# refresh-bio/fqsqueezer

Hardware: AMD Instinct MI355X
Metric: Mbases/s compressed (DNA stream, SE sorted) (higher is better)
Workload: dtype u64; 1 GPU; 1000000x150bp SE, G=7500000 (seed 2+rank), -om s -gs 8 -qm n -im n; workers_T=64, blocks=256, per_gpu=one independent file per GPU

## Files before the change

### fqsqueezer_amd/csrc/fqsx_api.hip

```cpp
#include "fqsx_kernels.h"
#include "fqsx_qual.h"
#include "fqsx_qdec.h"
#include "../../include/fqsx.h"
#include "fqsx_vm.h"
#include "fqsx_rt.h"
#include <sys/resource.h>

#ifndef FQSX_EMU
#include <dlfcn.h>
#include <rccl/rccl.h>
#endif
#include <algorithm>
#include <cstdio>
#include <cstdlib>
#include <cstring>
#include <string>
#include <vector>

extern "C" const char *fqsx_last_error(void) { return g_err.c_str(); }
extern "C" const char *fqsx_version(void) {
#ifdef FQSX_EMU
  return "fqsx 0.1 (host emulation build - tests only)";
#else
  return "fqsx 0.1 (HIP gfx950)";
// ... 30 lines not shown
    for (u64 i = first; i < nb_slots; i += stride) cfg.l_b.slots[i] = 0;
    for (u64 i = first; i < ns_slots; i += stride) cfg.l_s.slots[i] = 0;
    for (u64 i = first; i < 2ull * cfg.T; i += stride) cfg.l_s.filled[i] = 0;
    return;
  }
  insert_phase_body(cfg, &sm, FQ_BLOCK / 3, FQ_BLOCK % 3, win, maxmult, by_source != 0);
  if (cfg.sys_scope) fq_release_system();
}
FQ_KERNEL64 void k_compact_generic(const u8 *out, u64 out_cap, const u64 *lens, u8 *dst) {
  const u32 tid = FQ_BLOCK;
  u64 off = 0;
  for (u32 t = 0; t < tid; ++t) off += lens[t];
  const u64 n = lens[tid] <= out_cap ? lens[tid] : 0;
  const u8 *src = out + (u64)tid * out_cap;
  for (u64 i = FQ_LANE; i < n; i += FQ_WAVE) dst[off + i] = src[i];
}
FQ_KERNEL64 void k_clear_local(DevCfg cfg, u64 nb_slots, u64 ns_slots) {
  if (phase_skip(cfg)) return;
  const u64 stride = (u64)FQ_NBLOCKS * FQ_WAVE, first = (u64)FQ_BLOCK * FQ_WAVE + FQ_LANE;
  for (u64 i = first; i < nb_slots; i += stride) cfg.l_b.slots[i] = 0;
  for (u64 i = first; i < ns_slots; i += stride) cfg.l_s.slots[i] = 0;
  for (u64 i = first; i < 2ull * cfg.T; i += stride) cfg.l_s.filled[i] = 0;
}
FQ_KERNEL64 void k_finish_block(DevCfg cfg, u64 *lens , u64 *end ) {
  if (FQ_LANE == 0) {
    if (FQ_BLOCK == 0) { end[2 * cfg.T] = cfg.err[0]; end[2 * cfg.T + 1] = cfg.err[1]; }
    if (cfg.err[1]) return;
    finish_block_body(cfg, FQ_BLOCK);
    lens[FQ_BLOCK] = cfg.ws[FQ_BLOCK].out_len;
    end[FQ_BLOCK] = cfg.ws[FQ_BLOCK].out_len;
// ... 467 lines not shown
    u8 *va = nullptr;
    u64 va_bytes = 0, chunk_bytes = 0;
    std::vector<fqsx_vm::Handle> h;
    std::vector<u8> mapped;
    u64 own_bytes = 0;
    u32 own_mod = 0;
    bool live = false;
  } vm_s, vm_b, vm_pk, vm_pv, vm_siv;
  u32 *d_plog_n;
  u32 ins_win, ins_maxmult;
  bool part_sender;
  bool defer_coding;
  u64 gq_entries;
  u32 gq_test_cap;
  bool cur_defer;
  u64 vm_own_bytes;
};

namespace {

#define FQSX_PIN_BYTES (64u * 1024u)
int d2h_small_begin(fqsx_dna *c, const void *d, u64 bytes) { return d2h(c, c->h_pin, d, bytes); }
int d2h_small_end(fqsx_dna *c, void *h, u64 bytes) {
  DEVCHK(dev_sync(c));
  memcpy(h, c->h_pin, bytes);
  return FQSX_OK;
}

#define REHASH_GRID FQ_GRID(2048)

// ... 347 lines not shown
  int rc = dev_launch(c, 0, true, [&] {
#ifndef FQSX_EMU
    if (defer) return fqsx_launch_encode_se_defer(c->stream, a);
#endif
    return decode ? fqsx_launch_decode(c->stream, a) : c->paired ? fqsx_launch_encode_pe(c->stream, a) : fqsx_launch_encode_se(c->stream, a);
  });
#ifndef FQSX_EMU
  if (!rc && defer) {
    if (c->profiling) rc = dev_launch(c, 2, true, [&] { return fqsx_launch_code_se(c->stream, a); });
    else if (!(rc = dev_side_launch(c, buf, [&] { return fqsx_launch_code_se(c->side, a); }))) c->k_n[2] += 1;
  }
#endif
  return rc;
}

int block_prepare(fqsx_dna *c, const u8 *d_bases, const u64 *d_off, const u64 *h_off, u32 n_reads, u32 generation,
                  const u8 *const *dec_streams = nullptr, const u64 *dec_lens = nullptr) {
  const bool decode = dec_streams != nullptr;
  const u32 T = c->T;
  DevCfg &cfg = c->cfg;
  u64 S = generation < 100u ? 100u - generation : 0u;
  u64 cap_s = (u64)n_reads / T / 2;
  if (S > cap_s) S = cap_s;
  if (S) --S;
  u64 max_wbases = 0, max_seg_bases = 0, max_seg_reads = 0, max_wreads = 0, max_defer_entries = 0;
  DEVCHK(dev_side_join(c));
  std::vector<u64> wbases(T);
  for (u32 t = 0; t < T; ++t) {
    u64 first, last;
    worker_reads(t, T, n_reads, first, last);
    wbases[t] = h_off[last] - h_off[first];
    max_wbases = std::max(max_wbases, wbases[t]);
// ... 5 lines not shown
        const u64 ns = segment_synchro(seg, S, first, last);
        if (!c->paired) stop = ns + 1;
        else { u64 i = cur; if (i < ns) i += (ns - i + 1) & ~1ull; stop = i + 2; }
      }
      if (stop > last) stop = last;
      if (stop > cur) {
        max_seg_bases = std::max(max_seg_bases, h_off[stop] - h_off[cur]);
        max_seg_reads = std::max(max_seg_reads, stop - cur);
        if (seg < S) max_defer_entries = std::max(max_defer_entries, h_off[stop] - h_off[cur] + (stop - cur) * (FQSX_HD_RAW + 0u));
        cur = stop;
      }
    }
  }
  int rc;
  void *p = nullptr;
  if (c->paired && (n_reads & 1)) { g_err = "paired-end blocks need an even number of reads"; return FQSX_E_ARG; }
  u64 need_out = max_wbases + 16 * max_wreads + 1024;
  if ((rc = dfit(c, cfg.out, cfg.out_cap, need_out, pow2_at_least(need_out), T))) return rc;
  const u64 mail_entries[3] = {2 * max_seg_bases + 2 * max_seg_reads, max_seg_bases, 2 * max_seg_bases};
  for (u32 k = 0; k < 3; ++k) {
    u64 need = mail_entries[k] + 64;
    if (need > c->mail_cap[k] && (rc = mail_alloc(c, k, (u32)(need + need / 4)))) return rc;
  }
  u64 need_lb = pow2_at_least(4 * max_seg_bases + 64), need_ls = pow2_at_least(2 * max_seg_bases + 64);
  if ((rc = ltab_fit(c, cfg.l_b, c->lb_cap, need_lb, cfg.bmer, 6))) return rc;
  if ((rc = ltab_fit(c, cfg.l_s, c->ls_cap, need_ls, cfg.smer, 12))) return rc;
  u64 need_lpe = 0;
  if (c->paired) {
    const u64 seg_pairs = max_seg_reads / 2 + 1;
    const u64 need_list = 14 * seg_pairs + 16;
    const u32 list_cap = (u32)(need_list + need_list / 4);
    if ((rc = dfit(c, cfg.pe_bkt, c->pe_bkt_cap, need_list, list_cap, (u64)T * 3 * sizeof(u64)))) return rc;
    if ((rc = dfit(c, cfg.pe_list, cfg.pe_cap, need_list, list_cap, (u64)T * 3 * sizeof(u64)))) return rc;
// ... 152 lines not shown
int pe_insert_and_clear(fqsx_dna *c) {
  LAUNCH(c, 2, k_pe_insert, c->T, 64, c->cfg);
  return pe_clear_local(c);
}

int block_segment(fqsx_dna *c, u32 seg) {
  const u32 T = c->T, n_reads = c->cur_n_reads;
  const u64 S = c->cur_S, need_lpe = c->cur_need_lpe;
  const bool decode = c->cur_decode;
  DevCfg &cfg = c->cfg;
  int rc;
  {
    const bool defer = c->cur_defer && seg < S;
    if (!defer) DEVCHK(dev_side_join(c));
    if ((rc = launch_segment(c, decode, n_reads, (u32)S, seg, defer))) return rc;
    const u32 part_grid = T * (cfg.mail[0].n_tiles + cfg.mail[1].n_tiles + cfg.mail[2].n_tiles);
    if (!decode && c->part_sender) LAUNCH(c, 2, k_part_sender, 3 * T, FQSX_SND_THREADS, cfg);
    else {
      LAUNCH(c, 2, k_part_count, part_grid, 64, cfg);
      LAUNCH(c, 2, k_part_scan, 3 * T, 64, cfg);
      if (!decode) LAUNCH(c, 2, k_part_scatter, part_grid, 64, cfg, seg + 1, c->d_demand);
    }
    if (!decode) {
      if (c->paired) {
        const u32 bgrid = FQ_GRID((u32)std::min<u64>(1024, ((u64)T * cfg.pe_cap + 255) / 256));
        LAUNCH(c, 2, k_pe_bucket_count, bgrid, 256, cfg);
        LAUNCH(c, 2, k_pe_bucket_offsets, 1, 64, cfg, seg + 1);
        LAUNCH(c, 2, k_pe_bucket_scatter, bgrid, 256, cfg);
        LAUNCH(c, 2, k_pe_insert_buckets, T, 64, cfg);
        if ((rc = pe_clear_local(c))) return rc;
// ... 8 lines not shown
      g_err = "device error " + std::to_string(c->h_demand[2 * T]) + " in decode kernel (block " + std::to_string(c->cur_gen) + ")";
      return FQSX_E_DEVICE;
    }
    if ((rc = grow_for_demand(c))) return rc;
    if (c->paired) {
      LAUNCH(c, 2, k_pe_demand, T, 64, cfg, c->d_demand, 0u);
      if ((rc = d2h_sync(c, c->h_demand.data(), c->d_demand, T * sizeof(u32)))) return rc;
      if ((rc = d2h_sync(c, c->h_filled.data(), cfg.g_pe.filled, T * sizeof(u32)))) return rc;
      u64 need = 0;
      for (u32 o = 0; o < T; ++o) need = std::max<u64>(need, (u64)c->h_filled[o] + c->h_demand[o]);
      if (need * 2 > c->gpe_cap && (rc = grow_gpe(c, pow2_at_least(need * 2 + 2)))) return rc;
      if ((rc = pe_insert_and_clear(c))) return rc;
    }
    LAUNCH(c, 1, k_insert_phase, 3 * T, FQSX_INS_THREADS, cfg, (u64)0, (u64)0, c->ins_win, c->ins_maxmult, 0u, 0u);
    if ((rc = clear_local_tables(c))) return rc;
  }
  return FQSX_OK;
}

int block_finish(fqsx_dna *c, const u64 *h_off, const u8 **streams, u64 *lens, u8 *bases_out, u32 *posted = nullptr) {
  if (posted) *posted = 0;
  const u32 T = c->T, n_reads = c->cur_n_reads, generation = c->cur_gen;
  const bool decode = c->cur_decode;
  DevCfg &cfg = c->cfg;
  int rc;
  if (decode) {
    u32 derr = 0;
    if ((rc = d2h_sync(c, &derr, cfg.err, sizeof(u32)))) return rc;
    if (derr) {
      g_err = "device error " + std::to_string(derr) + " while decoding block " + std::to_string(generation);
      return FQSX_E_DEVICE;
    }
    return bases_out ? d2h_sync(c, bases_out, cfg.dout, h_off[n_reads]) : FQSX_OK;
  }
  DEVCHK(dev_side_join(c));
  LAUNCH(c, 2, k_finish_block, T, 64, cfg, c->d_lens, c->d_end);
  {
    std::vector<u64> e(2 * T + 2);
    if ((rc = d2h_small_begin(c, c->d_end, e.size() * sizeof(u64)))) return rc;
    if ((rc = d2h_small_end(c, e.data(), e.size() * sizeof(u64)))) return rc;
    if (e[2 * T]) {
      g_err = "device error " + std::to_string(e[2 * T]) + " while encoding block " + std::to_string(generation);
      return FQSX_E_DEVICE;
    }
    if (e[2 * T + 1]) {
      if (posted) { *posted = (u32)e[2 * T + 1]; return FQSX_OK; }
      g_err = "growth posted by the device outside the deferred path";
      return FQSX_E_DEVICE;
    }
    for (u32 t = 0; t < T; ++t) { c->h_lens[t] = e[t]; c->h_filled[t] = (u32)e[T + t]; }
    c->filled_valid = true;
  }
  u64 total = 0;
  for (u32 t = 0; t < T; ++t) {
    if (c->h_lens[t] > cfg.out_cap) { g_err = "stream overflow"; return FQSX_E_DEVICE; }
    total += c->h_lens[t];
  }
  if ((rc = dfit(c, c->d_compact, c->compact_cap, total, total + total / 2 + 4096, 1))) return rc;
  return collect_streams(c, c->d_compact, T, cfg.out, cfg.out_cap, c->d_lens, c->h_lens, c->h_out, streams, lens);
}

int encode_block_impl(fqsx_dna *c, const u8 *d_bases, const u64 *d_off, const u64 *h_off, u32 n_reads, u32 generation,
                      const u8 **streams, u64 *lens, const u8 *const *dec_streams = nullptr, const u64 *dec_lens = nullptr,
                      u8 *bases_out = nullptr) {
  if (c->shard_world > 1) { g_err = "a sharded codec is driven through fqsx_shard_* (fqsqueezer_amd/sharded.py)"; return FQSX_E_ARG; }
  int rc = block_prepare(c, d_bases, d_off, h_off, n_reads, generation, dec_streams, dec_lens);
  for (u32 seg = 0; !rc;) {
    for (; !rc && seg <= c->cur_S; ++seg) rc = block_segment(c, seg);
    u32 posted = 0;
    if (!rc) rc = block_finish(c, h_off, streams, lens, bases_out, &posted);
    if (rc || !posted) break;
    rc = block_recover(c, posted - 1);
    seg = posted;
  }
  return rc;
}

bool defer_possible(fqsx_dna *c, u32 n_parts) {
#ifdef FQSX_EMU
  (void)c; (void)n_parts;
  return false;
// ... 134 lines not shown
  }
  cfg.shard_rank = 0; cfg.shard_world = 1; cfg.shard_cnt = nullptr;
  if ((rc = dalloc(c, &p, sizeof(u32) * 4, true))) return rc;
  cfg.err = (u32 *)p;
#ifdef FQSX_TIMING
  if ((rc = dalloc(c, &p, (u64)FQSX_TRACE_LAUNCHES * T * FQSX_TRACE_W * sizeof(u64), true))) return rc;
  cfg.trace = (u64 *)p;
#endif
  if ((rc = dalloc(c, &p, (5 * (u64)T + 2) * sizeof(u32), true))) return rc;
  c->d_demand = cfg.demand = (u32 *)p;
  if ((rc = dalloc(c, &p, ((u64)T + 64) * sizeof(u64), true))) return rc;
  c->d_lens = (u64 *)p;
  if ((rc = dalloc(c, &p, (2 * (u64)T + 2) * sizeof(u64), true))) return rc;
  c->d_end = (u64 *)p;
  if ((rc = pinned_alloc((void **)&c->h_pin, FQSX_PIN_BYTES))) return rc;
  c->h_demand.assign(4 * T + 1, 0);
  c->h_filled.assign(T, 0);
  c->h_lens.assign(T + 64, 0);
  DEVCHK(dev_sync(c));
  return FQSX_OK;
}

}

extern "C" {

int fqsx_dna_create(const uint8_t *h, int device, fqsx_dna **out) { return fqsx_dna_create_on_partition(h, device, 0, 1, out); }

int fqsx_dna_create_on_partition(const uint8_t *h, int device, uint32_t part, uint32_t n_parts, fqsx_dna **out) {
  if (n_parts == 0 || part >= n_parts) { g_err = "bad compute-unit partition"; return FQSX_E_ARG; }
// ... 16 lines not shown
  }
  rc = create_impl(c, h);
  if (!rc) c->defer_coding = defer_possible(c, n_parts);
  if (!rc && getenv("FQSX_CHUNKED_TABLES") && atoi(getenv("FQSX_CHUNKED_TABLES"))) rc = fqsx_dna_use_chunked_tables(c);
  if (rc) {
    fqsx_dna_destroy(c);
    return rc;
  }
  *out = c;
  return FQSX_OK;
}

void fqsx_dna_destroy(fqsx_dna *c) {
  if (!c) return;
  dev_close(c);
  vtab_free(c, c->vm_s);
  vtab_free(c, c->vm_b);
  vtab_free(c, c->vm_pk);
  vtab_free(c, c->vm_pv);
  vtab_free(c, c->vm_siv);
  fqsx_vm::mesh_close(c->mesh);
  pinned_free(c->h_pin);
  delete c;
}

int fqsx_dna_encode_block_dev(fqsx_dna *c, const uint8_t *d_bases, const uint64_t *d_off, const uint64_t *h_off,
                              uint32_t n_reads, uint32_t generation, const uint8_t **streams, uint64_t *lens) {
  if (!c || !d_bases || !d_off || !h_off || !streams || !lens) { g_err = "null argument"; return FQSX_E_ARG; }
  DEVCHK(dev_enter(c));
  return encode_block_impl(c, d_bases, d_off, h_off, n_reads, generation, streams, lens);
}

int fqsx_dna_encode_block(fqsx_dna *c, const uint8_t *bases, const uint64_t *off, uint32_t n_reads, uint32_t generation,
                          const uint8_t **streams, uint64_t *lens) {
  if (!c || !bases || !off || !streams || !lens) { g_err = "null argument"; return FQSX_E_ARG; }
  DEVCHK(dev_enter(c));
  int rc;
  u64 nb = off[n_reads] + 64, no = ((u64)n_reads + 1) * sizeof(u64);
  if ((rc = dfit(c, c->d_bases, c->dev_bases_cap, nb, nb + nb / 4, 1))) return rc;
  if ((rc = dfit(c, c->d_off, c->dev_off_cap, no, no + no / 4, 1))) return rc;
  if ((rc = h2d(c, c->d_bases, bases, off[n_reads]))) return rc;
  if ((rc = h2d(c, c->d_off, off, no))) return rc;
  return encode_block_impl(c, c->d_bases, c->d_off, off, n_reads, generation, streams, lens);
}

static int decode_args_ok(const fqsx_dna *c, const uint8_t *const *streams, const uint64_t *lens, const uint64_t *off, uint32_t n_reads) {
  if (c->paired && (n_reads & 1)) { g_err = "paired-end blocks need an even number of reads"; return FQSX_E_ARG; }
  if (off[0] != 0) { g_err = "read offsets do not start at 0"; return FQSX_E_ARG; }
  for (uint32_t i = 0; i < n_reads; ++i) {
    if (off[i + 1] < off[i]) { g_err = "read offsets do not ascend"; return FQSX_E_ARG; }
    if (off[i + 1] - off[i] >= (1ull << 24)) { g_err = "a read of 2^24 bases or more"; return FQSX_E_ARG; }
  }
  for (uint32_t t = 0; t < c->T; ++t)
    if (lens[t] && !streams[t]) { g_err = "null stream"; return FQSX_E_ARG; }
  return FQSX_OK;
}

int fqsx_dna_decode_block(fqsx_dna *c, const uint8_t *const *streams, const uint64_t *lens, const uint64_t *off, uint32_t n_reads,
                          uint32_t generation, uint8_t *bases_out) {
  if (!c || !streams || !lens || !off || !bases_out) { g_err = "null argument"; return FQSX_E_ARG; }
  if (int bad = decode_args_ok(c, streams, lens, off, n_reads)) return bad;
  DEVCHK(dev_enter(c));
  int rc;
  u64 no = ((u64)n_reads + 1) * sizeof(u64);
  if ((rc = dfit(c, c->d_off, c->dev_off_cap, no, no + no / 4, 1))) return rc;
  if ((rc = h2d(c, c->d_off, off, no))) return rc;
  return encode_block_impl(c, nullptr, c->d_off, off, n_reads, generation, nullptr, nullptr, streams, lens, bases_out);
}

int fqsx_dna_decode_block_dev(fqsx_dna *c, const uint8_t *const *streams, const uint64_t *lens, const uint64_t *off, uint32_t n_reads,
                              uint32_t generation, const uint8_t **d_bases_out) {
  if (d_bases_out) *d_bases_out = nullptr;
  if (!c || !streams || !lens || !off || !d_bases_out) { g_err = "null argument"; return FQSX_E_ARG; }
  if (int bad = decode_args_ok(c, streams, lens, off, n_reads)) return bad;
  DEVCHK(dev_enter(c));
  int rc;
  u64 no = ((u64)n_reads + 1) * sizeof(u64);
  if ((rc = dfit(c, c->d_off, c->dev_off_cap, no, no + no / 4, 1))) return rc;
  if ((rc = h2d(c, c->d_off, off, no))) return rc;
  if ((rc = encode_block_impl(c, nullptr, c->d_off, off, n_reads, generation, nullptr, nullptr, streams, lens, nullptr))) return rc;
  *d_bases_out = c->cfg.dout;
  return FQSX_OK;
}

int fqsx_shard_config(fqsx_dna *c, uint32_t rank, uint32_t world) {
  if (!c || world == 0 || rank >= world || world > c->T) { g_err = "bad rank / world size"; return FQSX_E_ARG; }
  if (c->part && world > 1) { g_err = "a codec with chunked tables cannot be sharded afterwards (fqsx_shard_partition_tables after the attach)"; return FQSX_E_ARG; }
  DEVCHK(dev_enter(c));
  const u32 T = c->T;
  c->shard_rank = rank; c->shard_world = world;
  c->cfg.shard_rank = rank; c->cfg.shard_world = world;
  u8 vm[256];
  for (u32 i = 0; i < 256; ++i) vm[i] = (u8)i;
  u32 v = 0;
  for (u32 q = 0; q < world; ++q)
    for (u32 o = q; o < T; o += world) vm[o] = (u8)v++;
  int rc;
  void *p = nullptr;
  if ((rc = h2d(c, c->d_vmap, vm, 256))) return rc;
  if (!c->cfg.shard_cnt) {
    if ((rc = dalloc(c, &p, (3ull * T * T + T + 1) * sizeof(u32), true))) return rc;
    c->cfg.shard_cnt = (u32 *)p;
    if ((rc = dalloc(c, &p, (3ull * T * T + T + 1) * sizeof(u32), true))) return rc;
// ... 1 lines not shown
    if ((rc = dalloc(c, &p, 3ull * (T + 1) * T * sizeof(u32), true))) return rc;
    c->d_colsum = (u32 *)p;
    if ((rc = dalloc(c, &p, 8 * sizeof(u64), true))) return rc;
    c->d_small = (u64 *)p;
    c->h_cglob.assign(3ull * T * T + T + 1, 0);
  }
  DEVCHK(dev_sync(c));
  return FQSX_OK;
}

int fqsx_shard_begin_block(fqsx_dna *c, const uint8_t *bases , const uint64_t *off , const uint64_t *h_off,
                           uint32_t n_reads, uint32_t generation, uint32_t *n_segments) {
  if (!c || !bases || !off || !h_off || !n_segments) { g_err = "null argument"; return FQSX_E_ARG; }
  if (c->part) { g_err = "partitioned tables are driven through fqsx_shard_encode_block"; return FQSX_E_ARG; }
  if (c->paired && c->shard_world > 1) { g_err = "paired-end files are sharded through fqsx_shard_attach + fqsx_shard_encode_block (the step-wise fqsx_shard_* driver does not exchange the pair-table triples)"; return FQSX_E_ARG; }
  DEVCHK(dev_enter(c));
  int rc = block_prepare(c, bases, off, h_off, n_reads, generation);
  *n_segments = c->cur_S + 1;
  return rc;
}

int fqsx_shard_encode(fqsx_dna *c, uint32_t seg, uint32_t *counts ) {
  if (!c || !counts) { g_err = "null argument"; return FQSX_E_ARG; }
  DEVCHK(dev_enter(c));
  const u32 T = c->T;
  DevCfg &cfg = c->cfg;
  int rc;
  if ((rc = launch_segment(c, false, c->cur_n_reads, c->cur_S, seg))) return rc;
  const u32 part_grid = T * (cfg.mail[0].n_tiles + cfg.mail[1].n_tiles + cfg.mail[2].n_tiles);
  LAUNCH(c, 2, k_part_count, part_grid, 64, cfg);
  LAUNCH(c, 2, k_shard_counts, 3 * T + 1, 64, cfg, cfg.shard_cnt, 0u);
  if ((rc = d2d(c, counts, cfg.shard_cnt, 3ull * T * T * sizeof(u32)))) return rc;
  u32 err = 0;
  if ((rc = d2h_sync(c, &err, cfg.err, sizeof(u32)))) return rc;
  if (err) { g_err = "device error " + std::to_string(err) + " in encode kernel"; return FQSX_E_DEVICE; }
  return FQSX_OK;
}

int fqsx_shard_pack(fqsx_dna *c, const uint32_t *counts_sum , uint64_t *const send[3] ) {
  if (!c || !counts_sum || !send) { g_err = "null argument"; return FQSX_E_ARG; }
  DEVCHK(dev_enter(c));
  const u32 T = c->T;
  DevCfg &cfg = c->cfg;
  int rc;
  if ((rc = d2d(c, c->d_cglob, counts_sum, 3ull * T * T * sizeof(u32)))) return rc;
  const u32 part_grid = T * (cfg.mail[0].n_tiles + cfg.mail[1].n_tiles + cfg.mail[2].n_tiles);
  LAUNCH(c, 2, k_part_scan, 3 * T, 64, cfg);
  LAUNCH(c, 2, k_part_dstoff, 3, 64, cfg, c->d_demand, 0u);
  LAUNCH(c, 2, k_part_scatter, part_grid, 64, cfg, 0u, (u32 *)nullptr);
  std::vector<u32> tot(3 * (T + 1));
  for (u32 k = 0; k < 3; ++k)
    if ((rc = d2h_sync(c, tot.data() + k * (T + 1), cfg.mail[k].dst_off, (T + 1) * sizeof(u32)))) return rc;
  for (u32 k = 0; k < 3; ++k) {
    const u64 n = tot[k * (T + 1) + T];
    if (n && (rc = d2d(c, send[k], cfg.mail[k].sorted, n * sizeof(u64)))) return rc;
  }
  DEVCHK(dev_sync(c));
  return FQSX_OK;
}

int fqsx_shard_merge(fqsx_dna *c, const uint64_t *const recv[3] , uint64_t need[2]) {
  if (!c || !recv || !need) { g_err = "null argument"; return FQSX_E_ARG; }
  DEVCHK(dev_enter(c));
  const u32 T = c->T;
  DevCfg &cfg = c->cfg;
  int rc;
  for (u32 k = 0; k < 3; ++k) LAUNCH(c, 2, k_shard_merge, T, 64, cfg, k, recv[k], (const u32 *)c->d_cglob);
  need[0] = need[1] = 0;
  std::vector<u32> tot(T), fil(T);
  for (int which = 0; which < 2; ++which) {
    const KTab &t = which ? cfg.g_b : cfg.g_s;
    if ((rc = d2h_sync(c, tot.data(), cfg.mail[which ? MAIL_B : MAIL_S].dst_tot, T * sizeof(u32)))) return rc;
    if ((rc = d2h_sync(c, fil.data(), t.filled, T * sizeof(u32)))) return rc;
    for (u32 o = 0; o < T; ++o) need[which] = std::max<u64>(need[which], (u64)tot[o] + fil[o]);
  }
  return FQSX_OK;
}

int fqsx_shard_insert(fqsx_dna *c, uint64_t need_s, uint64_t need_b, uint64_t *const items[3] , uint64_t siv_delta[2]) {
  if (!c || !items || !siv_delta) { g_err = "null argument"; return FQSX_E_ARG; }
  DEVCHK(dev_enter(c));
  const u32 T = c->T;
  DevCfg &cfg = c->cfg;
  int rc;
  if (tab_over(c, need_s, c->gs_cap) && (rc = grow_global(c, cfg.g_s, c->gs_cap, tab_new_cap(c, need_s)))) return rc;
  if (tab_over(c, need_b, c->gb_cap) && (rc = grow_global(c, cfg.g_b, c->gb_cap, tab_new_cap(c, need_b)))) return rc;
  if ((rc = d2h_sync(c, c->siv_before, cfg.siv_stats, 2 * sizeof(u64)))) return rc;
  LAUNCH(c, 1, k_insert_phase, 3 * T, FQSX_INS_THREADS, cfg, (u64)0, (u64)0, c->ins_win, c->ins_maxmult, 0u, 0u);
  u64 after[2];
  if ((rc = d2h_sync(c, after, cfg.siv_stats, 2 * sizeof(u64)))) return rc;
  siv_delta[0] = after[0] - c->siv_before[0];
  siv_delta[1] = after[1] - c->siv_before[1];
  for (u32 k = 0; k < 3; ++k) LAUNCH(c, 2, k_shard_collect, REHASH_GRID, 256, cfg, k, items[k]);
  DEVCHK(dev_sync(c));
  return FQSX_OK;
}

int fqsx_shard_apply(fqsx_dna *c, uint32_t kind, const uint64_t *items , uint64_t n) {
  if (!c || kind > 2 || (!items && n)) { g_err = "bad argument"; return FQSX_E_ARG; }
  DEVCHK(dev_enter(c));
  if (n) LAUNCH(c, 2, k_shard_apply, REHASH_GRID, 256, c->cfg, kind, items, (u32)n);
  return FQSX_OK;
}

int fqsx_shard_end_phase(fqsx_dna *c, const uint64_t siv_delta_sum[2]) {
  if (!c || !siv_delta_sum) { g_err = "null argument"; return FQSX_E_ARG; }
  DEVCHK(dev_enter(c));
  int rc;
  u64 now[2] = {c->siv_before[0] + siv_delta_sum[0], c->siv_before[1] + siv_delta_sum[1]};
  if ((rc = h2d(c, c->cfg.siv_stats, now, 2 * sizeof(u64)))) return rc;
  DEVCHK(dev_sync(c));
  return clear_local_tables(c);
}

int fqsx_shard_finish_block(fqsx_dna *c, const uint64_t *h_off, const uint8_t **streams, uint64_t *lens) {
  if (!c || !h_off || !streams || !lens) { g_err = "null argument"; return FQSX_E_ARG; }
  DEVCHK(dev_enter(c));
  return block_finish(c, h_off, streams, lens, nullptr);
}

namespace {
int xbuf_fit(fqsx_dna *c, u64 *&buf, u64 &cap, u64 words) { return dfit(c, buf, cap, words, words + words / 4 + 1024, sizeof(u64)); }
#define COMMCHK(x, what) do { if ((x) != 0) { if (g_err.empty() || g_err.find(what) == std::string::npos) g_err = std::string(what) + " failed"; if (c->comm.abort) c->comm.abort(c->comm.ctx); return FQSX_E_HIP; } } while (0)

int shard_vote(fqsx_dna *c, int fail, const char *what) {
  const u64 NC = 3ull * c->T * c->T + c->T + 1;
  u32 *word = c->d_cglob + NC - 1;
  u32 v = fail ? 1u : 0u;
  const std::string mine = g_err;
  int rc;
  if ((rc = h2d(c, word, &v, sizeof(v)))) return rc;
  DEVCHK(dev_sync(c));
// ... 181 lines not shown
      c->cfg.siv = (u64 *)c->vm_siv.va;
      c->cfg.siv_part = 1;
      void *p = nullptr;
      if ((rc = dalloc(c, &p, 2 * sizeof(u32), true))) return rc;
      c->d_plog_n = (u32 *)p;
      c->cfg.p_log_n = c->d_plog_n;
    }
  }
  DEVCHK(dev_sync(c));
  return FQSX_OK;
}
}

int fqsx_dna_use_chunked_tables(fqsx_dna *c) {
  if (!c) { g_err = "null argument"; return FQSX_E_ARG; }
  if (c->part) return FQSX_OK;
  if (c->k_n[0] || c->shard_world > 1) { g_err = "chunked tables are chosen before the first block (sharded codecs: fqsx_shard_partition_tables)"; return FQSX_E_ARG; }
  DEVCHK(dev_enter(c));
  return tables_to_chunks(c);
}

int fqsx_shard_partition_tables(fqsx_dna *c) {
  if (!c || !c->comm_set) { g_err = "no transport attached (fqsx_shard_attach)"; return FQSX_E_ARG; }
  if (c->part && (c->shard_world == 1 || !c->mesh.peer.empty())) return FQSX_OK;
  if (c->part || c->k_n[0]) { g_err = "the tables can only be partitioned before the first block"; return FQSX_E_ARG; }
  DEVCHK(dev_enter(c));
  const u32 G = c->shard_world, me = c->shard_rank;
  int rc;
  c->part_fallback = false;
#ifndef FQSX_EMU
  if (G > 1) {
    u64 mine[2] = {0, 0};
    char bus[16] = {0};
    HIPCHK(hipDeviceGetPCIBusId(bus, (int)sizeof(bus), c->device));
    memcpy(mine, bus, sizeof(mine));
    std::vector<u64> all(2ull * G, 0);
    if ((rc = xbuf_fit(c, c->d_items, c->items_cap, 2))) return rc;
    if ((rc = xbuf_fit(c, c->d_gathered, c->gathered_cap, 2ull * G))) return rc;
    if ((rc = h2d(c, c->d_items, mine, sizeof(mine)))) return rc;
    DEVCHK(dev_sync(c));
    COMMCHK(c->comm.allgather_u64(c->comm.ctx, c->d_items, 2, c->d_gathered), "all-gather of the ranks' PCI bus ids");
// ... 27 lines not shown
  if ((rc = xbuf_fit(c, c->d_gathered, c->gathered_cap, G))) return rc;
  if ((rc = h2d(c, c->d_items, &c->mesh.word, sizeof(u64)))) return rc;
  COMMCHK(c->comm.allgather_u64(c->comm.ctx, c->d_items, 1, c->d_gathered), "all-gather of the descriptor-socket names");
  if ((rc = d2h_sync(c, words.data(), c->d_gathered, G * sizeof(u64)))) return rc;
  VMCHK(fqsx_vm::mesh_connect(c->mesh, words.data(), e_));
  if ((rc = tables_to_chunks(c))) return rc;
  COMMCHK(c->comm.allgather_u64(c->comm.ctx, c->d_items, 1, c->d_gathered), "barrier after the table partition");
  DEVCHK(dev_sync(c));
  return FQSX_OK;
}

int fqsx_shard_encode_block(fqsx_dna *c, const uint8_t *bases, const uint64_t *off, const uint64_t *h_off, uint32_t n_reads,
                            uint32_t generation, const uint8_t **streams, uint64_t *lens) {
  if (!c || !bases || !off || !h_off || !streams || !lens) { g_err = "null argument"; return FQSX_E_ARG; }
  if (!c->comm_set) { g_err = "no transport attached (fqsx_shard_attach)"; return FQSX_E_ARG; }
  DEVCHK(dev_enter(c));
  int rc = block_prepare(c, bases, off, h_off, n_reads, generation);
  for (u32 seg = 0; !rc && seg <= c->cur_S; ++seg) rc = shard_phase_native(c, seg);
  if (rc) return rc;
  return block_finish(c, h_off, streams, lens, nullptr);
}

int fqsx_shard_is_partitioned(fqsx_dna *c) { return c && c->part && !c->part_fallback ? 1 : 0; }

int fqsx_shard_traffic(fqsx_dna *c, uint64_t out[4]) {
  if (!c || !out) return FQSX_E_ARG;
  out[0] = c->sh_phases; out[1] = c->sh_collectives; out[2] = c->sh_a2a_words; out[3] = c->sh_gather_words;
  return FQSX_OK;
}

#ifndef FQSX_EMU
namespace {
struct RcclApi {
  void *lib = nullptr;
  ncclResult_t (*GetUniqueId)(ncclUniqueId *) = nullptr;
  ncclResult_t (*CommInitRank)(ncclComm_t *, int, ncclUniqueId, int) = nullptr;
  ncclResult_t (*CommDestroy)(ncclComm_t) = nullptr;
  ncclResult_t (*CommAbort)(ncclComm_t) = nullptr;
  ncclResult_t (*CommCount)(const ncclComm_t, int *) = nullptr;
  ncclResult_t (*CommUserRank)(const ncclComm_t, int *) = nullptr;
  ncclResult_t (*AllReduce)(const void *, void *, size_t, ncclDataType_t, ncclRedOp_t, ncclComm_t, hipStream_t) = nullptr;
// ... 51 lines not shown
}
}

int fqsx_rccl_unique_id(uint8_t id[128]) {
  if (!id) return FQSX_E_ARG;
  if (!rccl_load()) return FQSX_E_HIP;
  static_assert(sizeof(ncclUniqueId) == 128, "ncclUniqueId is 128 bytes");
  ncclUniqueId u;
  if (g_rccl.GetUniqueId(&u) != ncclSuccess) { g_err = "ncclGetUniqueId failed"; return FQSX_E_HIP; }
  memcpy(id, &u, 128);
  return FQSX_OK;
}
int fqsx_rccl_comm_create(fqsx_dna *c, const uint8_t id[128], uint32_t rank, uint32_t world, fqsx_comm *out) {
  if (!c || !id || !out || world == 0 || rank >= world) { g_err = "bad argument"; return FQSX_E_ARG; }
  if (!rccl_load()) return FQSX_E_HIP;
  DEVCHK(dev_enter(c));
  ncclUniqueId u;
  memcpy(&u, id, 128);
  RcclCtx *x = new RcclCtx();
  x->stream = c->stream;
  x->world = world;
  x->aborted = false;
  ncclResult_t r = g_rccl.CommInitRank(&x->comm, (int)world, u, (int)rank);
  if (r != ncclSuccess) { g_err = std::string("ncclCommInitRank: ") + g_rccl.GetErrorString(r); delete x; return FQSX_E_HIP; }
  out->ctx = x;
  out->allreduce_sum_u32 = rccl_allreduce;
  out->alltoallv_u64 = rccl_alltoallv;
  out->allgather_u64 = rccl_allgather;
  out->abort = rccl_abort;
  return FQSX_OK;
}
int fqsx_rccl_comm_rebind(fqsx_comm *m, fqsx_dna *c) {
  if (!m || !m->ctx || !c) { g_err = "bad argument"; return FQSX_E_ARG; }
  ((RcclCtx *)m->ctx)->stream = c->stream;
  return FQSX_OK;
}
int fqsx_rccl_comm_info(fqsx_comm *m, uint32_t out[2]) {
  if (!m || !m->ctx || !out) { g_err = "bad argument"; return FQSX_E_ARG; }
  RcclCtx *x = (RcclCtx *)m->ctx;
  int n = 0, r = 0;
  if (g_rccl.CommCount(x->comm, &n) != ncclSuccess || g_rccl.CommUserRank(x->comm, &r) != ncclSuccess) { g_err = "ncclCommCount / ncclCommUserRank failed"; return FQSX_E_HIP; }
  out[0] = (u32)n; out[1] = (u32)r;
  return FQSX_OK;
}
void fqsx_rccl_comm_destroy(fqsx_comm *m) {
  if (!m || !m->ctx) return;
  RcclCtx *x = (RcclCtx *)m->ctx;
  if (g_rccl.CommDestroy && !x->aborted) (void)g_rccl.CommDestroy(x->comm);
  delete x;
  m->ctx = nullptr;
}
#else
static int no_rccl() { g_err = "the emulation build has no RCCL transport"; return FQSX_E_NO_DEVICE; }
int fqsx_rccl_unique_id(uint8_t *) { return no_rccl(); }
int fqsx_rccl_comm_create(fqsx_dna *, const uint8_t *, uint32_t, uint32_t, fqsx_comm *) { return no_rccl(); }
int fqsx_rccl_comm_rebind(fqsx_comm *, fqsx_dna *) { return no_rccl(); }
int fqsx_rccl_comm_info(fqsx_comm *, uint32_t *) { return no_rccl(); }
void fqsx_rccl_comm_destroy(fqsx_comm *) {}
#endif

int fqsx_dna_stats(fqsx_dna *c, uint64_t out[64]) {
  if (!c || !out) return FQSX_E_ARG;
  DEVCHK(dev_enter(c));
  LAUNCH(c, 2, k_gather_stats, 1, 64, c->cfg, c->d_lens + c->T);
  return d2h_sync(c, out, c->d_lens + c->T, 64 * sizeof(u64));
}

int fqsx_dna_capacity(fqsx_dna *c, uint64_t out[16]) {
  if (!c || !out) return FQSX_E_ARG;
  DEVCHK(dev_enter(c));
  const u32 T = c->T;
  std::vector<u32> f(T);
  int rc;
  for (int i = 0; i < 16; ++i) out[i] = 0;
  if ((rc = d2h_sync(c, f.data(), c->cfg.g_s.filled, T * sizeof(u32)))) return rc;
  for (u32 t = 0; t < T; ++t) out[0] += f[t];
  if ((rc = d2h_sync(c, f.data(), c->cfg.g_b.filled, T * sizeof(u32)))) return rc;
  for (u32 t = 0; t < T; ++t) out[1] += f[t];
  out[2] = c->gs_cap * T;
  out[3] = c->gb_cap * T;
  out[4] = (1ull << (2 * c->cfg.pmer)) / 4;
  out[5] = c->ctx_cap * T;
  if ((rc = d2h_sync(c, f.data(), c->cfg.ctx_filled, T * sizeof(u32)))) return rc;
  for (u32 t = 0; t < T; ++t) out[6] += f[t];
  out[7] = c->dev_bytes;
// ... 1 lines not shown
  out[9] = c->n_growths;
  if (c->paired) {
    if ((rc = d2h_sync(c, f.data(), c->cfg.g_pe.filled, T * sizeof(u32)))) return rc;
    for (u32 t = 0; t < T; ++t) out[10] += f[t];
    out[11] = c->gpe_cap * T;
  }
  out[12] = sizeof(u64);
  out[13] = (c->vm_s.live ? c->vm_s.own_bytes : c->gs_cap * T * sizeof(u64)) + (c->vm_b.live ? c->vm_b.own_bytes : c->gb_cap * T * sizeof(u64));
  out[15] = c->vm_siv.live ? c->vm_siv.own_bytes : out[4];
  if (c->paired) out[14] = c->vm_pk.live ? c->vm_pk.own_bytes + c->vm_pv.own_bytes : c->gpe_cap * T * 2 * sizeof(u64);
  return FQSX_OK;
}

static_assert(FQSX_TRACE_WORDS == FQSX_TRACE_W, "include/fqsx.h documents the trace record width");
int fqsx_dna_trace(fqsx_dna *c, uint64_t *out, uint32_t max_launches) {
  if (!c || !out || !c->cfg.trace) return 0;
  u32 n = (u32)std::min<u64>(std::min<u64>(c->k_n[0], FQSX_TRACE_LAUNCHES), max_launches);
  if (n && d2h_sync(c, out, c->cfg.trace, (u64)n * c->T * FQSX_TRACE_W * sizeof(u64))) return 0;
  return (int)n;
}

int fqsx_dna_set_profiling(fqsx_dna *c, int enable) {
  if (!c) return FQSX_E_ARG;
  if (c->side_last >= 0) { DEVCHK(dev_enter(c)); DEVCHK(dev_sync(c)); }
  c->profiling = enable != 0;
  return FQSX_OK;
}
int fqsx_dna_kernel_times(fqsx_dna *c, double out[6]) {
  if (!c || !out) return FQSX_E_ARG;
  for (int i = 0; i < 3; ++i) { out[i] = c->k_ms[i]; out[3 + i] = (double)c->k_n[i]; }
  return FQSX_OK;
}

}

FQ_KERNEL64 void k_qual_encode(QualCfg cfg, u32 n_reads) {
  FQ_SHARED u8 lds_q[4096 + 96];
  qual_encode_body(cfg, lds_q, FQ_BLOCK, n_reads);
}
FQ_KERNEL64 void k_qual_decode(QualCfg cfg, QualDecArgs da, u32 n_reads) { qual_decode_body(cfg, da, FQ_BLOCK, n_reads); }
FQ_KERNEL void k_qual_rehash(const u64 *o, u64 ocap_mask, u64 *n, u64 ncap_mask, u32 T, u32 slot_u64) {
  const u64 ocap = ocap_mask + 1, total = ocap * T;
  const u64 gstride = FQ_GRID_STRIDE(u64);
  for (u64 g = FQ_GRID_FIRST(u64); g < total; g += gstride) {
// ... 1452 lines not shown
```

### fqsqueezer_amd/csrc/fqsx_rt.h

```cpp
#pragma once
#include "fqsx_plat.h"
#include "../../include/fqsx.h"
#include <algorithm>
#include <cstdlib>
#include <cstring>
#include <string>
#include <vector>

static thread_local std::string g_err;

#ifndef FQSX_EMU
typedef hipStream_t DevStream;
typedef hipEvent_t DevEvent;
#else
typedef void *DevStream;
typedef void *DevEvent;
#endif

struct DevCtx {
  int device = 0;
  DevStream stream = nullptr;
  DevEvent ev0 = nullptr, ev1 = nullptr;
  bool profiling = false;
  DevStream side = nullptr;
// ... 127 lines not shown
static int d2d(DevCtx *c, void *d, const void *s, u64 bytes) {
  HIPCHK(hipMemcpyAsync(d, s, bytes, hipMemcpyDeviceToDevice, c->stream));
  return FQSX_OK;
}
static int d2h(DevCtx *c, void *h, const void *d, u64 bytes) {
  HIPCHK(hipMemcpyAsync(h, d, bytes, hipMemcpyDeviceToHost, c->stream));
  return FQSX_OK;
}
static int pinned_alloc(void **p, u64 bytes) {
  HIPCHK(hipHostMalloc(p, bytes));
  return FQSX_OK;
}
static void pinned_free(void *p) {
  if (p) (void)hipHostFree(p);
}
static void dev_drain(DevCtx *c) {
  (void)hipSetDevice(c->device);
  (void)hipStreamSynchronize(c->stream);
  if (c->side) (void)hipStreamSynchronize(c->side);
  c->side_used[0] = c->side_used[1] = false;
  c->side_last = -1;
}
static void dev_destroy_stream(DevCtx *c) {
  (void)hipEventDestroy(c->ev0);
  (void)hipEventDestroy(c->ev1);
  (void)hipStreamDestroy(c->stream);
  dev_side_close(c);
}
template <class F> static int dev_launch(DevCtx *c, u32 kidx, bool count, F &&launch) {
  if (c->profiling) HIPCHK(hipEventRecord(c->ev0, c->stream));
// ... 32 lines not shown
}
static int h2d(DevCtx *, void *d, const void *h, u64 bytes) {
  memcpy(d, h, bytes);
  return FQSX_OK;
}
static int d2d(DevCtx *, void *d, const void *s, u64 bytes) {
  memcpy(d, s, bytes);
  return FQSX_OK;
}
static int d2h(DevCtx *, void *h, const void *d, u64 bytes) {
  memcpy(h, d, bytes);
  return FQSX_OK;
}
static int pinned_alloc(void **p, u64 bytes) { return dev_malloc(p, bytes); }
static void pinned_free(void *p) { free(p); }
static void dev_drain(DevCtx *) {}
static void dev_destroy_stream(DevCtx *) {}
template <class F> static int dev_launch(DevCtx *c, u32 kidx, bool, F &&launch) {
  launch();
  c->k_n[kidx] += 1;
  return FQSX_OK;
}
template <class F> static int emu_grid(u32 grid, F &&block) {
  fq_emu_nblocks = grid;
  for (u32 b = 0; b < grid; ++b) {
    fq_emu_block = b;
    block();
  }
  return 0;
}
// ... 66 lines not shown
```

Measured before the change: 121.6 Mbases/s.

## Defer last-phase table inserts past stream readback for single-GPU SE encode

For single-GPU single-end encoding, the last segment no longer runs its part-sender/insert/clear before finishing the block. Instead, finish and a new fused compact kernel (which also copies the end/error header) are launched, and the streams are read into a pinned slab with one D2H sized from the previous block. The last phase's inserts are then queued behind an event, and the host returns streams without waiting for them. Pending inserts are settled (error and growth checks) at the next API entry, which adds event bookkeeping and deferred error reporting.

```diff
diff --git a/fqsqueezer_amd/csrc/fqsx_api.hip b/fqsqueezer_amd/csrc/fqsx_api.hip
--- a/fqsqueezer_amd/csrc/fqsx_api.hip
+++ b/fqsqueezer_amd/csrc/fqsx_api.hip
@@ -68,6 +68,20 @@
   const u64 n = lens[tid] <= out_cap ? lens[tid] : 0;
   const u8 *src = out + (u64)tid * out_cap;
   for (u64 i = FQ_LANE; i < n; i += FQ_WAVE) dst[off + i] = src[i];
+}
+FQ_KERNEL64 void k_compact_end(const u8 *out, u64 out_cap, const u64 *lens, const u64 *end, u32 T, u8 *dst, u64 room) {
+  const u32 tid = FQ_BLOCK;
+  if (tid == 0)
+    for (u32 i = FQ_LANE; i < 2 * T + 2; i += FQ_WAVE) ((u64 *)dst)[i] = end[i];
+  if (end[2 * T] | end[2 * T + 1]) return;
+  u64 off = 0;
+  for (u32 t = 0; t < tid; ++t) off += lens[t];
+  u64 n = lens[tid] <= out_cap ? lens[tid] : 0;
+  if (off >= room) n = 0;
+  else if (n > room - off) n = room - off;
+  const u8 *src = out + (u64)tid * out_cap;
+  u8 *to = dst + (2 * (u64)T + 2) * sizeof(u64) + off;
+  for (u64 i = FQ_LANE; i < n; i += FQ_WAVE) to[i] = src[i];
 }
 FQ_KERNEL64 void k_clear_local(DevCfg cfg, u64 nb_slots, u64 ns_slots) {
   if (phase_skip(cfg)) return;
@@ -565,6 +579,14 @@
   u64 gq_entries;
   u32 gq_test_cap;
   bool cur_defer;
+  bool late_insert, cur_late;
+  bool tail_pending;
+  u32 tail_gen;
+  DevEvent ev_streams, ev_tail;
+  u32 *h_tail_err;
+  u8 *h_slab;
+  u64 slab_cap, slab_hint;
+  u64 slab_test_cap;
   u64 vm_own_bytes;
 };
 
@@ -942,8 +964,9 @@
   return rc;
 }
 
+int tail_settle(fqsx_dna *c);
 int block_prepare(fqsx_dna *c, const u8 *d_bases, const u64 *d_off, const u64 *h_off, u32 n_reads, u32 generation,
-                  const u8 *const *dec_streams = nullptr, const u64 *dec_lens = nullptr) {
+                  const u8 *const *dec_streams = nullptr, const u64 *dec_lens = nullptr, bool late_ok = false) {
   const bool decode = dec_streams != nullptr;
   const u32 T = c->T;
   DevCfg &cfg = c->cfg;
@@ -979,9 +1002,22 @@
   }
   int rc;
   void *p = nullptr;
+  if ((rc = tail_settle(c))) return rc;
   if (c->paired && (n_reads & 1)) { g_err = "paired-end blocks need an even number of reads"; return FQSX_E_ARG; }
   u64 need_out = max_wbases + 16 * max_wreads + 1024;
   if ((rc = dfit(c, cfg.out, cfg.out_cap, need_out, pow2_at_least(need_out), T))) return rc;
+  const bool se_one_gpu = late_ok && !decode && !c->paired && c->part_sender && c->shard_world == 1;
+  c->cur_late = se_one_gpu && c->late_insert;
+  if (se_one_gpu) {
+    const u64 need = (2 * (u64)T + 2) * sizeof(u64) + T * need_out;
+    if ((rc = dfit(c, c->d_compact, c->compact_cap, need, need + need / 4, 1))) return rc;
+    if (c->cur_late && need > c->slab_cap) {
+      pinned_free(c->h_slab);
+      c->h_slab = nullptr; c->slab_cap = 0;
+      if ((rc = pinned_alloc((void **)&c->h_slab, need + need / 4))) return rc;
+      c->slab_cap = need + need / 4;
+    }
+  }
   const u64 mail_entries[3] = {2 * max_seg_bases + 2 * max_seg_reads, max_seg_bases, 2 * max_seg_bases};
   for (u32 k = 0; k < 3; ++k) {
     u64 need = mail_entries[k] + 64;
@@ -1164,6 +1200,7 @@
     const bool defer = c->cur_defer && seg < S;
     if (!defer) DEVCHK(dev_side_join(c));
     if ((rc = launch_segment(c, decode, n_reads, (u32)S, seg, defer))) return rc;
+    if (c->cur_late && seg == S) return FQSX_OK;
     const u32 part_grid = T * (cfg.mail[0].n_tiles + cfg.mail[1].n_tiles + cfg.mail[2].n_tiles);
     if (!decode && c->part_sender) LAUNCH(c, 2, k_part_sender, 3 * T, FQSX_SND_THREADS, cfg);
     else {
@@ -1202,6 +1239,80 @@
     }
     LAUNCH(c, 1, k_insert_phase, 3 * T, FQSX_INS_THREADS, cfg, (u64)0, (u64)0, c->ins_win, c->ins_maxmult, 0u, 0u);
     if ((rc = clear_local_tables(c))) return rc;
+  }
+  return FQSX_OK;
+}
+
+int tail_drop(fqsx_dna *c) {
+  if (!c->tail_pending) return FQSX_OK;
+  c->tail_pending = false;
+  return dev_event_wait(c->ev_tail);
+}
+int tail_settle(fqsx_dna *c) {
+  if (!c->tail_pending) return FQSX_OK;
+  c->tail_pending = false;
+  DEVCHK(dev_event_wait(c->ev_tail));
+  const u32 err = c->h_tail_err[0], posted = c->h_tail_err[1];
+  const std::string where = "the last phase's inserts of block " + std::to_string(c->tail_gen);
+  if (err) { g_err = "device error " + std::to_string(err) + " in " + where; return FQSX_E_DEVICE; }
+  if (!posted) return FQSX_OK;
+  if (posted != c->cur_S + 1) { g_err = "phase " + std::to_string(posted - 1) + " posted for growth by " + where; return FQSX_E_DEVICE; }
+  const int rc = block_recover(c, c->cur_S);
+  if (rc) g_err += " (" + where + ")";
+  return rc;
+}
+int dna_enter(fqsx_dna *c) {
+  DEVCHK(dev_enter(c));
+  return tail_settle(c);
+}
+int block_finish_late(fqsx_dna *c, const u8 **streams, u64 *lens, u32 *posted) {
+  const u32 T = c->T;
+  DevCfg &cfg = c->cfg;
+  int rc;
+  const u64 hdr = (2 * (u64)T + 2) * sizeof(u64), room = std::min(c->compact_cap, c->slab_cap) - hdr;
+  LAUNCH(c, 2, k_finish_block, T, 64, cfg, c->d_lens, c->d_end);
+  LAUNCH(c, 2, k_compact_end, T, 64, cfg.out, cfg.out_cap, c->d_lens, c->d_end, T, c->d_compact, room);
+  u64 slab = std::max<u64>(c->slab_hint + c->slab_hint / 4, 64u * 1024u);
+  if (c->slab_test_cap) slab = std::min(slab, c->slab_test_cap - 1);
+  slab = std::min(slab, room);
+  if ((rc = d2h(c, c->h_slab, c->d_compact, hdr + slab))) return rc;
+  DEVCHK(dev_event_record(c, c->ev_streams));
+  LAUNCH(c, 2, k_part_sender, 3 * T, FQSX_SND_THREADS, cfg);
+  if ((rc = insert_and_clear(c, c->cur_S + 1))) return rc;
+  if ((rc = d2h(c, c->h_tail_err, cfg.err, 2 * sizeof(u32)))) return rc;
+  DEVCHK(dev_event_record(c, c->ev_tail));
+  c->tail_pending = true;
+  c->tail_gen = c->cur_gen;
+  if ((rc = dev_event_wait(c->ev_streams))) { (void)tail_drop(c); return rc; }
+  const u64 *e = (const u64 *)c->h_slab;
+  if (e[2 * T]) {
+    (void)tail_drop(c);
+    g_err = "device error " + std::to_string(e[2 * T]) + " while encoding block " + std::to_string(c->cur_gen);
+    return FQSX_E_DEVICE;
+  }
+  if (e[2 * T + 1]) {
+    DEVCHK(tail_drop(c));
+    if (posted) { *posted = (u32)e[2 * T + 1]; return FQSX_OK; }
+    g_err = "growth posted by the device outside the deferred path";
+    return FQSX_E_DEVICE;
+  }
+  u64 total = 0;
+  for (u32 t = 0; t < T; ++t) {
+    if (e[t] > cfg.out_cap || e[t] > room - total) { (void)tail_drop(c); g_err = "stream overflow"; return FQSX_E_DEVICE; }
+    total += e[t];
+  }
+  for (u32 t = 0; t < T; ++t) { c->h_lens[t] = e[t]; c->h_filled[t] = (u32)e[T + t]; }
+  c->filled_valid = true;
+  c->slab_hint = total;
+  if (total > slab) {
+    if ((rc = d2h(c, c->h_slab + hdr + slab, c->d_compact + hdr + slab, total - slab))) return rc;
+    DEVCHK(dev_sync(c));
+  }
+  u64 pos = hdr;
+  for (u32 t = 0; t < T; ++t) {
+    streams[t] = c->h_slab + pos;
+    lens[t] = e[t];
+    pos += e[t];
   }
   return FQSX_OK;
 }
@@ -1222,6 +1333,7 @@
     return bases_out ? d2h_sync(c, bases_out, cfg.dout, h_off[n_reads]) : FQSX_OK;
   }
   DEVCHK(dev_side_join(c));
+  if (c->cur_late) return block_finish_late(c, streams, lens, posted);
   LAUNCH(c, 2, k_finish_block, T, 64, cfg, c->d_lens, c->d_end);
   {
     std::vector<u64> e(2 * T + 2);
@@ -1252,7 +1364,7 @@
                       const u8 **streams, u64 *lens, const u8 *const *dec_streams = nullptr, const u64 *dec_lens = nullptr,
                       u8 *bases_out = nullptr) {
   if (c->shard_world > 1) { g_err = "a sharded codec is driven through fqsx_shard_* (fqsqueezer_amd/sharded.py)"; return FQSX_E_ARG; }
-  int rc = block_prepare(c, d_bases, d_off, h_off, n_reads, generation, dec_streams, dec_lens);
+  int rc = block_prepare(c, d_bases, d_off, h_off, n_reads, generation, dec_streams, dec_lens, true);
   for (u32 seg = 0; !rc;) {
     for (; !rc && seg <= c->cur_S; ++seg) rc = block_segment(c, seg);
     u32 posted = 0;
@@ -1417,6 +1529,12 @@
   if ((rc = dalloc(c, &p, (2 * (u64)T + 2) * sizeof(u64), true))) return rc;
   c->d_end = (u64 *)p;
   if ((rc = pinned_alloc((void **)&c->h_pin, FQSX_PIN_BYTES))) return rc;
+  if ((rc = pinned_alloc((void **)&c->h_tail_err, 64))) return rc;
+  c->h_tail_err[0] = c->h_tail_err[1] = 0;
+  DEVCHK(dev_event_open(&c->ev_streams));
+  DEVCHK(dev_event_open(&c->ev_tail));
+  c->late_insert = !(getenv("FQSX_LATE_INSERT") && atoi(getenv("FQSX_LATE_INSERT")) == 0);
+  if (const char *e = getenv("FQSX_TEST_SLAB")) c->slab_test_cap = strtoull(e, nullptr, 10) + 1;
   c->h_demand.assign(4 * T + 1, 0);
   c->h_filled.assign(T, 0);
   c->h_lens.assign(T + 64, 0);
@@ -1463,6 +1581,11 @@
 void fqsx_dna_destroy(fqsx_dna *c) {
   if (!c) return;
   dev_close(c);
+  c->tail_pending = false;
+  dev_event_close(c->ev_streams);
+  dev_event_close(c->ev_tail);
+  pinned_free(c->h_tail_err);
+  pinned_free(c->h_slab);
   vtab_free(c, c->vm_s);
   vtab_free(c, c->vm_b);
   vtab_free(c, c->vm_pk);
@@ -1483,7 +1606,7 @@
 int fqsx_dna_encode_block(fqsx_dna *c, const uint8_t *bases, const uint64_t *off, uint32_t n_reads, uint32_t generation,
                           const uint8_t **streams, uint64_t *lens) {
   if (!c || !bases || !off || !streams || !lens) { g_err = "null argument"; return FQSX_E_ARG; }
-  DEVCHK(dev_enter(c));
+  DEVCHK(dna_enter(c));
   int rc;
   u64 nb = off[n_reads] + 64, no = ((u64)n_reads + 1) * sizeof(u64);
   if ((rc = dfit(c, c->d_bases, c->dev_bases_cap, nb, nb + nb / 4, 1))) return rc;
@@ -1509,7 +1632,7 @@
                           uint32_t generation, uint8_t *bases_out) {
   if (!c || !streams || !lens || !off || !bases_out) { g_err = "null argument"; return FQSX_E_ARG; }
   if (int bad = decode_args_ok(c, streams, lens, off, n_reads)) return bad;
-  DEVCHK(dev_enter(c));
+  DEVCHK(dna_enter(c));
   int rc;
   u64 no = ((u64)n_reads + 1) * sizeof(u64);
   if ((rc = dfit(c, c->d_off, c->dev_off_cap, no, no + no / 4, 1))) return rc;
@@ -1522,7 +1645,7 @@
   if (d_bases_out) *d_bases_out = nullptr;
   if (!c || !streams || !lens || !off || !d_bases_out) { g_err = "null argument"; return FQSX_E_ARG; }
   if (int bad = decode_args_ok(c, streams, lens, off, n_reads)) return bad;
-  DEVCHK(dev_enter(c));
+  DEVCHK(dna_enter(c));
   int rc;
   u64 no = ((u64)n_reads + 1) * sizeof(u64);
   if ((rc = dfit(c, c->d_off, c->dev_off_cap, no, no + no / 4, 1))) return rc;
@@ -1535,7 +1658,7 @@
 int fqsx_shard_config(fqsx_dna *c, uint32_t rank, uint32_t world) {
   if (!c || world == 0 || rank >= world || world > c->T) { g_err = "bad rank / world size"; return FQSX_E_ARG; }
   if (c->part && world > 1) { g_err = "a codec with chunked tables cannot be sharded afterwards (fqsx_shard_partition_tables after the attach)"; return FQSX_E_ARG; }
-  DEVCHK(dev_enter(c));
+  DEVCHK(dna_enter(c));
   const u32 T = c->T;
   c->shard_rank = rank; c->shard_world = world;
   c->cfg.shard_rank = rank; c->cfg.shard_world = world;
@@ -1567,7 +1690,7 @@
   if (!c || !bases || !off || !h_off || !n_segments) { g_err = "null argument"; return FQSX_E_ARG; }
   if (c->part) { g_err = "partitioned tables are driven through fqsx_shard_encode_block"; return FQSX_E_ARG; }
   if (c->paired && c->shard_world > 1) { g_err = "paired-end files are sharded through fqsx_shard_attach + fqsx_shard_encode_block (the step-wise fqsx_shard_* driver does not exchange the pair-table triples)"; return FQSX_E_ARG; }
-  DEVCHK(dev_enter(c));
+  DEVCHK(dna_enter(c));
   int rc = block_prepare(c, bases, off, h_off, n_reads, generation);
   *n_segments = c->cur_S + 1;
   return rc;
@@ -1575,7 +1698,7 @@
 
 int fqsx_shard_encode(fqsx_dna *c, uint32_t seg, uint32_t *counts ) {
   if (!c || !counts) { g_err = "null argument"; return FQSX_E_ARG; }
-  DEVCHK(dev_enter(c));
+  DEVCHK(dna_enter(c));
   const u32 T = c->T;
   DevCfg &cfg = c->cfg;
   int rc;
@@ -1592,7 +1715,7 @@
 
 int fqsx_shard_pack(fqsx_dna *c, const uint32_t *counts_sum , uint64_t *const send[3] ) {
   if (!c || !counts_sum || !send) { g_err = "null argument"; return FQSX_E_ARG; }
-  DEVCHK(dev_enter(c));
+  DEVCHK(dna_enter(c));
   const u32 T = c->T;
   DevCfg &cfg = c->cfg;
   int rc;
@@ -1614,7 +1737,7 @@
 
 int fqsx_shard_merge(fqsx_dna *c, const uint64_t *const recv[3] , uint64_t need[2]) {
   if (!c || !recv || !need) { g_err = "null argument"; return FQSX_E_ARG; }
-  DEVCHK(dev_enter(c));
+  DEVCHK(dna_enter(c));
   const u32 T = c->T;
   DevCfg &cfg = c->cfg;
   int rc;
@@ -1632,7 +1755,7 @@
 
 int fqsx_shard_insert(fqsx_dna *c, uint64_t need_s, uint64_t need_b, uint64_t *const items[3] , uint64_t siv_delta[2]) {
   if (!c || !items || !siv_delta) { g_err = "null argument"; return FQSX_E_ARG; }
-  DEVCHK(dev_enter(c));
+  DEVCHK(dna_enter(c));
   const u32 T = c->T;
   DevCfg &cfg = c->cfg;
   int rc;
@@ -1651,14 +1774,14 @@
 
 int fqsx_shard_apply(fqsx_dna *c, uint32_t kind, const uint64_t *items , uint64_t n) {
   if (!c || kind > 2 || (!items && n)) { g_err = "bad argument"; return FQSX_E_ARG; }
-  DEVCHK(dev_enter(c));
+  DEVCHK(dna_enter(c));
   if (n) LAUNCH(c, 2, k_shard_apply, REHASH_GRID, 256, c->cfg, kind, items, (u32)n);
   return FQSX_OK;
 }
 
 int fqsx_shard_end_phase(fqsx_dna *c, const uint64_t siv_delta_sum[2]) {
   if (!c || !siv_delta_sum) { g_err = "null argument"; return FQSX_E_ARG; }
-  DEVCHK(dev_enter(c));
+  DEVCHK(dna_enter(c));
   int rc;
   u64 now[2] = {c->siv_before[0] + siv_delta_sum[0], c->siv_before[1] + siv_delta_sum[1]};
   if ((rc = h2d(c, c->cfg.siv_stats, now, 2 * sizeof(u64)))) return rc;
@@ -1668,7 +1791,7 @@
 
 int fqsx_shard_finish_block(fqsx_dna *c, const uint64_t *h_off, const uint8_t **streams, uint64_t *lens) {
   if (!c || !h_off || !streams || !lens) { g_err = "null argument"; return FQSX_E_ARG; }
-  DEVCHK(dev_enter(c));
+  DEVCHK(dna_enter(c));
   return block_finish(c, h_off, streams, lens, nullptr);
 }
 
@@ -1880,17 +2003,17 @@
 
 int fqsx_dna_use_chunked_tables(fqsx_dna *c) {
   if (!c) { g_err = "null argument"; return FQSX_E_ARG; }
+  DEVCHK(dna_enter(c));
   if (c->part) return FQSX_OK;
   if (c->k_n[0] || c->shard_world > 1) { g_err = "chunked tables are chosen before the first block (sharded codecs: fqsx_shard_partition_tables)"; return FQSX_E_ARG; }
-  DEVCHK(dev_enter(c));
   return tables_to_chunks(c);
 }
 
 int fqsx_shard_partition_tables(fqsx_dna *c) {
   if (!c || !c->comm_set) { g_err = "no transport attached (fqsx_shard_attach)"; return FQSX_E_ARG; }
+  DEVCHK(dna_enter(c));
   if (c->part && (c->shard_world == 1 || !c->mesh.peer.empty())) return FQSX_OK;
   if (c->part || c->k_n[0]) { g_err = "the tables can only be partitioned before the first block"; return FQSX_E_ARG; }
-  DEVCHK(dev_enter(c));
   const u32 G = c->shard_world, me = c->shard_rank;
   int rc;
   c->part_fallback = false;
@@ -1948,7 +2071,7 @@
                             uint32_t generation, const uint8_t **streams, uint64_t *lens) {
   if (!c || !bases || !off || !h_off || !streams || !lens) { g_err = "null argument"; return FQSX_E_ARG; }
   if (!c->comm_set) { g_err = "no transport attached (fqsx_shard_attach)"; return FQSX_E_ARG; }
-  DEVCHK(dev_enter(c));
+  DEVCHK(dna_enter(c));
   int rc = block_prepare(c, bases, off, h_off, n_reads, generation);
   for (u32 seg = 0; !rc && seg <= c->cur_S; ++seg) rc = shard_phase_native(c, seg);
   if (rc) return rc;
@@ -1959,6 +2082,7 @@
 
 int fqsx_shard_traffic(fqsx_dna *c, uint64_t out[4]) {
   if (!c || !out) return FQSX_E_ARG;
+  DEVCHK(dna_enter(c));
   out[0] = c->sh_phases; out[1] = c->sh_collectives; out[2] = c->sh_a2a_words; out[3] = c->sh_gather_words;
   return FQSX_OK;
 }
@@ -2040,7 +2164,7 @@
 int fqsx_rccl_comm_create(fqsx_dna *c, const uint8_t id[128], uint32_t rank, uint32_t world, fqsx_comm *out) {
   if (!c || !id || !out || world == 0 || rank >= world) { g_err = "bad argument"; return FQSX_E_ARG; }
   if (!rccl_load()) return FQSX_E_HIP;
-  DEVCHK(dev_enter(c));
+  DEVCHK(dna_enter(c));
   ncclUniqueId u;
   memcpy(&u, id, 128);
   RcclCtx *x = new RcclCtx();
@@ -2058,6 +2182,7 @@
 }
 int fqsx_rccl_comm_rebind(fqsx_comm *m, fqsx_dna *c) {
   if (!m || !m->ctx || !c) { g_err = "bad argument"; return FQSX_E_ARG; }
+  DEVCHK(dna_enter(c));
   ((RcclCtx *)m->ctx)->stream = c->stream;
   return FQSX_OK;
 }
@@ -2087,14 +2212,14 @@
 
 int fqsx_dna_stats(fqsx_dna *c, uint64_t out[64]) {
   if (!c || !out) return FQSX_E_ARG;
-  DEVCHK(dev_enter(c));
+  DEVCHK(dna_enter(c));
   LAUNCH(c, 2, k_gather_stats, 1, 64, c->cfg, c->d_lens + c->T);
   return d2h_sync(c, out, c->d_lens + c->T, 64 * sizeof(u64));
 }
 
 int fqsx_dna_capacity(fqsx_dna *c, uint64_t out[16]) {
   if (!c || !out) return FQSX_E_ARG;
-  DEVCHK(dev_enter(c));
+  DEVCHK(dna_enter(c));
   const u32 T = c->T;
   std::vector<u32> f(T);
   int rc;
@@ -2126,7 +2251,7 @@
 
 static_assert(FQSX_TRACE_WORDS == FQSX_TRACE_W, "include/fqsx.h documents the trace record width");
 int fqsx_dna_trace(fqsx_dna *c, uint64_t *out, uint32_t max_launches) {
-  if (!c || !out || !c->cfg.trace) return 0;
+  if (!c || !out || !c->cfg.trace || dna_enter(c)) return 0;
   u32 n = (u32)std::min<u64>(std::min<u64>(c->k_n[0], FQSX_TRACE_LAUNCHES), max_launches);
   if (n && d2h_sync(c, out, c->cfg.trace, (u64)n * c->T * FQSX_TRACE_W * sizeof(u64))) return 0;
   return (int)n;
@@ -2134,12 +2259,14 @@
 
 int fqsx_dna_set_profiling(fqsx_dna *c, int enable) {
   if (!c) return FQSX_E_ARG;
-  if (c->side_last >= 0) { DEVCHK(dev_enter(c)); DEVCHK(dev_sync(c)); }
+  DEVCHK(dna_enter(c));
+  if (c->side_last >= 0) DEVCHK(dev_sync(c));
   c->profiling = enable != 0;
   return FQSX_OK;
 }
 int fqsx_dna_kernel_times(fqsx_dna *c, double out[6]) {
   if (!c || !out) return FQSX_E_ARG;
+  DEVCHK(dna_enter(c));
   for (int i = 0; i < 3; ++i) { out[i] = c->k_ms[i]; out[3 + i] = (double)c->k_n[i]; }
   return FQSX_OK;
 }
diff --git a/fqsqueezer_amd/csrc/fqsx_rt.h b/fqsqueezer_amd/csrc/fqsx_rt.h
--- a/fqsqueezer_amd/csrc/fqsx_rt.h
+++ b/fqsqueezer_amd/csrc/fqsx_rt.h
@@ -165,6 +165,21 @@
 static void pinned_free(void *p) {
   if (p) (void)hipHostFree(p);
 }
+static int dev_event_open(DevEvent *e) {
+  HIPCHK(hipEventCreateWithFlags(e, hipEventDisableTiming));
+  return FQSX_OK;
+}
+static int dev_event_record(DevCtx *c, DevEvent e) {
+  HIPCHK(hipEventRecord(e, c->stream));
+  return FQSX_OK;
+}
+static int dev_event_wait(DevEvent e) {
+  HIPCHK(hipEventSynchronize(e));
+  return FQSX_OK;
+}
+static void dev_event_close(DevEvent e) {
+  if (e) (void)hipEventDestroy(e);
+}
 static void dev_drain(DevCtx *c) {
   (void)hipSetDevice(c->device);
   (void)hipStreamSynchronize(c->stream);
@@ -227,6 +242,10 @@
 }
 static int pinned_alloc(void **p, u64 bytes) { return dev_malloc(p, bytes); }
 static void pinned_free(void *p) { free(p); }
+static int dev_event_open(DevEvent *) { return FQSX_OK; }
+static int dev_event_record(DevCtx *, DevEvent) { return FQSX_OK; }
+static int dev_event_wait(DevEvent) { return FQSX_OK; }
+static void dev_event_close(DevEvent) {}
 static void dev_drain(DevCtx *) {}
 static void dev_destroy_stream(DevCtx *) {}
 template <class F> static int dev_launch(DevCtx *c, u32 kidx, bool, F &&launch) {
```

After: 121.5 Mbases/s, median of 2. About the same (-0.0%).
